# Peer222/art-sbir

Measured on AMD Instinct MI355X. Metric: triplet-images/sec embedded @224² bf16, 1→8 GPU; gallery kNN QPS @1M×512, higher is better.
Workload: dtype bf16; 1 GPU; triplet training step (train.py:59-70): 3x encoder fwd + TripletMarginLoss + backward + Adam; model=ModifiedResNet((3,4,6,3), output_dim=512), global_batch=384, triplets_per_gpu=384, resolution=224, parallelism=dp1

## Files before the change

### art-sbir_amd/csrc/bstream.hip

```cpp
#include "common.h"
#include "pgemm.h"
#include "pgemm_dev.h"
#include "../../include/artsbir.h"

namespace artsbir {

constexpr int BS_NW = 8;
constexpr int BS_KC = 4;
constexpr int BS_CHUNK = 64;
constexpr int BS_NSEGT = 2;
#ifndef ARTSBIR_BS_NT
#define ARTSBIR_BS_NT 0
#endif

#define BS_GLOBAL __attribute__((address_space(1)))
template <typename T>
__device__ __forceinline__ BS_GLOBAL T* bs_base(T* p, long long off) {
  return (BS_GLOBAL T*)pg_uniform((long long)(p + off));
}

typedef __attribute__((ext_vector_type(4))) unsigned bs_u4;
template <bool NT>
__device__ __forceinline__ void bs_store(BS_GLOBAL bf16* p, const Vec16<bf16>& v) {
  if constexpr (NT) __builtin_nontemporal_store(*reinterpret_cast<const bs_u4*>(&v), reinterpret_cast<BS_GLOBAL bs_u4*>(p));
  else *reinterpret_cast<BS_GLOBAL bs_u4*>(p) = *reinterpret_cast<const bs_u4*>(&v);
}

struct BsArgs {
  const bf16* y3;
  const bf16* res;
  const bf16* w;
  const float* bn3;
  const float* bnd;
  bf16* out;
  unsigned char* bits;
  bf16* y1;
  float* stats;
  int nblk;
  int seg_blk;
  int nseg;
  int chunk;
};

template <int K, int N, bool TWO>
__global__ void __launch_bounds__(BS_NW * 64) bstream_kernel(BsArgs a) {
  constexpr int CPR = K / 8;
  constexpr int NKC = K / (32 * BS_KC);
  constexpr int NT = N / 16;
  constexpr int NP = N / 32;
  constexpr int NQ = TWO ? 6 : 3;
  static_assert(NKC % 2 == 0, "two operand sets, a whole number of pairs per block");
  __shared__ __attribute__((aligned(16))) char wlds[N * K * 2];
  __shared__ __attribute__((aligned(16))) float prm[BS_NSEGT][NQ][K];

  const int tid = threadIdx.x, lane = tid & 63;
  const int wid = __builtin_amdgcn_readfirstlane(tid >> 6);
  const int fr = lane & 15, fq = lane >> 4;
  const int b0 = blockIdx.x * a.chunk;
  const int b1 = b0 + a.chunk < a.nblk ? b0 + a.chunk : a.nblk;
// ... 258 lines not shown
```

### art-sbir_amd/csrc/gemm.hip

```cpp
#include <cstdio>
#include <cstdlib>
#include <tuple>
#include <vector>

#include "common.h"
#include "conv_launch.h"
#include "pgemm.h"
#include "tune.h"

namespace artsbir {

typedef __attribute__((ext_vector_type(4))) unsigned int u32x4;
#define OOB_OFFSET 0x80000000u

__device__ __forceinline__ __amdgpu_buffer_rsrc_t make_rsrc(const void* base, long long bytes) {
  if (bytes > 0x7fffffffLL) bytes = 0x7fffffffLL;
  if (bytes < 0) bytes = 0;
  return __builtin_amdgcn_make_buffer_rsrc(const_cast<void*>(base), (short)0, (int)bytes, 0x00020000);
}
__device__ __forceinline__ uint4 bload(__amdgpu_buffer_rsrc_t r, unsigned off) {
  u32x4 v = __builtin_amdgcn_raw_buffer_load_b128(r, (int)off, 0, 0);
  return make_uint4(v[0], v[1], v[2], v[3]);
}

// ... 668 lines not shown
  if (!g_tune_stats.reserve(bd ? per * bd->ntarget : (a.stats ? per : 0))) return pgemm_default_cfg(p);
  ConvArgs at = a;
  PgArgs pt = p;
  artsbir_bn_bwd_desc bt;
  if (a.stats) { at.stats = g_tune_stats.p; pt.stats = g_tune_stats.p; }
  if (bd) {
    bt = *bd;
    for (int t = 0; t < bd->ntarget; ++t) { bt.slots[t] = g_tune_stats.p + t * per; pt.bnb_slots[t] = bt.slots[t]; }
    at.bnb_desc = &bt;
  }
  return tune::fastest(pgemm_tune_candidates(), -2, st, [&](int c) { return run_candidate(c, at, pt, st); });
}

template <typename T>
static int launch_conv(const ConvArgs& a, hipStream_t st) {
  if ((long long)a.Cout * a.K * sizeof(T) > 0x7fffffffLL) { set_error("conv: weight tensor too large"); return -1; }
  if (a.nseg < 1 || a.M % a.nseg || (a.M / a.nseg) % ((long long)a.Ho * a.Wo)) {
    set_error("conv: %d BN segments do not split %lld output pixels into whole images", a.nseg, a.M);
    return -1;
  }
  const bool bnb = a.bnb_desc != nullptr;
  if (sizeof(T) == 2 && !a.out_f32 && !a.accumulate && !a.in_scale && !((a.bias || a.relu) && a.stats)) {
    const PgArgs p = to_pg(a);
    if (a.wg_p) {
      if (!pg_fold_wg_launch(p, st)) return 1;
      ARTSBIR_CHECK_LAUNCH("pgemm");
      return 0;
    }
    int choice;
    const char* force = getenv("ARTSBIR_PGEMM_CFG");
    static const char* force_bnb = getenv("ARTSBIR_BNB_CFG");
    if (force || (bnb && force_bnb)) {
      choice = atoi(force ? force : force_bnb);
    } else {
      const ConvKey key{a.M, a.H, a.W, a.C, a.Cout, a.R, a.S, a.stride, a.pad, a.Ho, a.Wo, a.res_mode,
                        (a.stats ? 1 : 0) | (a.bias ? 2 : 0) | (a.relu ? 4 : 0) | (a.x2 ? 8 : 0), a.nseg,
                        bnb ? p.bnb * 4 + p.bnb_nt : 0};
      choice = g_conv_choice.choice(
          key, st,
          [&] {
            const int c = pgemm_default_cfg(p);
            return c < 0 ? -2 : c;
          },
          [&] { return tune_conv(a, p, st); });
    }
    if ((choice != -2 && pgemm_launch_cfg(p, choice, st)) || (bnb && force_bnb && pgemm_launch_cfg(p, 0, st))) {
      ARTSBIR_CHECK_LAUNCH("pgemm");
      return 0;
    }
  }
  if (a.res_mode == 3) { set_error("gemm_nt_gate: no kernel for this shape"); return -1; }
  if (a.x2 || a.wg_p) return 1;
  return run_old<T>(a, st);
}

int artsbir::conv_launch(int dtype, const ConvArgs& a, hipStream_t st) {
  return dtype == ARTSBIR_DT_BF16 ? launch_conv<bf16>(a, st) : launch_conv<float>(a, st);
}

extern "C" int artsbir_conv2d_fwd(const artsbir_conv_desc* d, const void* x, const void* w, void* y,
                                  long long ldy, int out_f32, int accumulate, const float* bias,
                                  const float* in_scale, const float* in_shift, int in_relu,
                                  float* stats, void* stream) {
  if (check_conv(d)) return -1;
  if (accumulate && !out_f32) { set_error("conv: accumulate requires f32 output"); return -1; }
  ConvArgs a = conv_args_nhwc(d, x, w, y);
// ... 259 lines not shown
```

### art-sbir_amd/csrc/pgemm.h

```cpp
#pragma once
#include <hip/hip_runtime.h>

#include <vector>

namespace artsbir {

struct PgArgs {
  const void* x;
  long long x_elems;
  long long sN, sH, sW;
  int H, W, C;
  int R, S, stride, pad;
  int Ho, Wo;
  const void* w;
  int Cout, K;
  long long M;
  void* y;
  long long ldy;
  float* stats;
  long long seg_m;
  long long seg_stride;
  const void* res;
  int res_mode;
  const float* bias;
// ... 67 lines not shown
inline long long pg_ntiles(const PgArgs& a, int bpx, int bch) {
  return ((a.M + bpx - 1) / bpx) * ((a.Cout + bch - 1) / bch);
}

inline bool pg_supported(const PgArgs& a, bool& multi) {
  if (a.Cout % 32 != 0 || a.M <= 0) return false;
  if (a.C % 64 == 0) multi = false;
  else if (a.C == 8 || a.C == 16 || a.C == 32) multi = true;
  else return false;
  if (a.R * a.S > 32 || a.K % 8 != 0) return false;
  if ((long long)a.Cout * a.K * 2 > 0x7fffffffLL) return false;
  const long long HoWo = (long long)a.Ho * a.Wo;
  if (((256 + HoWo - 1) / HoWo + 2) * a.sN * 2 > 0x7fffffffLL) return false;
  if (a.M > (1LL << 40)) return false;
  if (a.seg_m > 0 && (a.seg_m % 64 != 0 || a.seg_m < 256 || a.M % a.seg_m != 0)) return false;
  if (a.bnb && (a.stats || a.Cout % 8 != 0)) return false;
  return true;
}

bool pg_pf_launch(int c, const PgArgs& a, bool multi, hipStream_t st);
bool pg_glb_launch(const PgArgs& a, bool multi, hipStream_t st);
bool pg_glb2_launch(const PgArgs& a, bool multi, hipStream_t st);
bool pg_k32w8_launch(const PgArgs& a, bool multi, hipStream_t st);
bool pg_fold_launch(const PgArgs& a, int c, hipStream_t st);
bool pstream_plain_launch(const PgArgs& a, bool multi, hipStream_t st);
bool pstream_bnb_launch(const PgArgs& a, bool multi, hipStream_t st);
bool pstream_k32_launch(const PgArgs& a, bool multi, hipStream_t st);
bool pstream_fold_launch(const PgArgs& a, int c, hipStream_t st);
bool sconv_launch(const PgArgs& a, hipStream_t st);
bool sconv_ok(const PgArgs& a);
bool hconv_launch(const PgArgs& a, hipStream_t st);
bool pp256_launch(const PgArgs& a, bool persistent, hipStream_t st);
bool rstream_launch(const PgArgs& a, hipStream_t st);
inline bool pg_fold_ok(const PgArgs& a, int bpx, int ks) {
  if (!a.x2 && !a.w_sstride) return true;
  if (a.R != 1 || a.S != 1 || a.stride != 1 || a.pad != 0) return false;
  if (a.x2 && (a.C1 <= 0 || a.C1 % ks != 0 || a.C1 >= a.C || (a.C - a.C1) % 8 != 0)) return false;
  if ((a.w_sstride || a.bias_sstride) && a.seg_m > 0 && a.seg_m % bpx != 0) return false;
  return true;
}
bool pg_fold_wg_launch(const PgArgs& a, hipStream_t st);
int pgemm_default_cfg(const PgArgs& a);

}
```

### art-sbir_amd/csrc/conv3x3.hip

```cpp
#include <cstdio>

#include "pgemm.h"
#include "pgemm_dev.h"

namespace artsbir {

__device__ __forceinline__ int sc_sw(int rho) { return (rho ^ (rho >> 1)) & 3; }

template <int C, int COUT, int STRIDE, bool BNB>
__global__ void __launch_bounds__(256) sconv_kernel(PgArgs a, int ntiles) {
  constexpr int K = 9 * C;
  constexpr int NKK = (K + 31) / 32;
  constexpr int CPT = C / 8;
  constexpr int MTC = COUT / 16, NTP = 4, WTPX = 64, BPX = 256, BCH = COUT;
  constexpr int PF = 2;
  constexpr int WB = NKK * COUT * 64;
  __shared__ __attribute__((aligned(16))) char smem[WB + pg_red_bytes<BCH>()];
  float* red = reinterpret_cast<float*>(smem + WB);
  int* red_cnt = reinterpret_cast<int*>(smem + WB + 6 * BCH * 4);
  const int tid = threadIdx.x, lane = tid & 63;
  const int wid = __builtin_amdgcn_readfirstlane(tid >> 6);
  const int fr = lane & 15, fq = lane >> 4;
  const bool sums = a.stats != nullptr || a.bnb != 0;
  if (sums) {
// ... 122 lines not shown
  } else if (a.stride == 1 && a.C == 32 && a.Cout == 64) {
    set_last_kernel(BNB ? "sconv_kernel<32,64,bnb>" : "sconv_kernel<32,64>");
    hipLaunchKernelGGL((sconv_kernel<32, 64, 1, BNB>), dim3(sconv_grid<32, 64, 1, BNB>(ntiles)), dim3(256), 0, st, a, ntiles);
  } else if (a.stride == 1 && a.C == 64 && a.Cout == 32) {
    set_last_kernel(BNB ? "sconv_kernel<64,32,bnb>" : "sconv_kernel<64,32>");
    hipLaunchKernelGGL((sconv_kernel<64, 32, 1, BNB>), dim3(sconv_grid<64, 32, 1, BNB>(ntiles)), dim3(256), 0, st, a, ntiles);
  } else if (a.stride == 1 && a.C == 64 && a.Cout == 64) {
    set_last_kernel(BNB ? "sconv_kernel<64,64,bnb>" : "sconv_kernel<64,64>");
    hipLaunchKernelGGL((sconv_kernel<64, 64, 1, BNB>), dim3(sconv_grid<64, 64, 1, BNB>(ntiles)), dim3(256), 0, st, a, ntiles);
  } else if (a.stride == 2 && a.C == 8 && a.Cout == 32) {
    set_last_kernel(BNB ? "sconv_kernel<8,32,s2,bnb>" : "sconv_kernel<8,32,s2>");
    hipLaunchKernelGGL((sconv_kernel<8, 32, 2, BNB>), dim3(sconv_grid<8, 32, 2, BNB>(ntiles)), dim3(256), 0, st, a, ntiles);
  } else {
    return false;
  }
  return true;
}

bool sconv_launch(const PgArgs& a, hipStream_t st) {
  if (!sconv_ok(a)) return false;
  const int ntiles = (int)((a.M + 255) / 256);
  if (a.bnb) return sconv_dispatch<true>(a, ntiles, st);
  return sconv_dispatch<false>(a, ntiles, st);
}

#define HC_MAXSEG 4
template <int C>
__device__ __forceinline__ int hc_addr(int q, int c) {
  constexpr int PB = 64 / (C / 8);
  constexpr int PBL = PB == 16 ? 4 : 3;
  return ((q >> PBL) << 10) + c * (PB * 16) + ((q & (PB - 1)) << 4);
}

template <int C, int COUT, int TR, int TC>
struct HcGeom {
  static constexpr int NWC = 4;
  static constexpr int CPT = C / 8, PB = 64 / CPT;
  static constexpr int NKK = 9 * C / 32;
  static constexpr int MTC = COUT / 16, NP = MTC / 2;
  static constexpr int TCB = TC / 16;
  static constexpr int NTP = TR * TCB / NWC;
  static constexpr int HW = TC + 2, NQ = HW * (TR + 2);
  static constexpr int NB = (NQ + PB - 1) / PB;
  static constexpr int HB = NB * 1024;
  static constexpr int WB = NKK * COUT * 64;
  static constexpr int PRM = HC_MAXSEG * 4 * COUT * 4;
  static constexpr int FIX = WB + PRM + pg_red_bytes<COUT>();
  static constexpr bool THREE = FIX + 3 * HB <= 160 * 1024 && (160 * 1024) / (FIX + 3 * HB) ==
                                (160 * 1024) / (FIX + 2 * HB) && NB <= 31;
  static constexpr int NBUF = THREE ? 3 : 2;
  static constexpr int LDS = WB + NBUF * HB + PRM + pg_red_bytes<COUT>();
  static constexpr int WPB = (160 * 1024) / LDS > 4 ? 4 : (160 * 1024) / LDS;
  static constexpr int WPE = (5 * WPB + 3) / 4 > 3 ? 3 : (5 * WPB + 3) / 4;
};

template <int C, int COUT, int TR, int TC, bool BNB>
__global__ void __launch_bounds__(320) __attribute__((amdgpu_waves_per_eu(HcGeom<C, COUT, TR, TC>::WPE)))
hconv_kernel(PgArgs a, int ntiles) {
  using Gm = HcGeom<C, COUT, TR, TC>;
  constexpr int NWC = Gm::NWC, PB = Gm::PB, NKK = Gm::NKK, MTC = Gm::MTC, NP = Gm::NP;
  constexpr int TCB = Gm::TCB, NTP = Gm::NTP, HW = Gm::HW, NQ = Gm::NQ, NB = Gm::NB, HB = Gm::HB;
  constexpr int WB = Gm::WB, NBUF = Gm::NBUF;
  static_assert(C % 32 == 0 && COUT % 32 == 0 && TC % 16 == 0, "tile shape");
  static_assert(NTP * NWC == TR * TCB, "pixel tiles per wave");
  static_assert(Gm::LDS <= 160 * 1024, "LDS");
  __shared__ __attribute__((aligned(16))) char smem[Gm::LDS];
  float* prm = reinterpret_cast<float*>(smem + WB + NBUF * HB);
  float* red = reinterpret_cast<float*>(smem + WB + NBUF * HB + Gm::PRM);
  int* red_cnt = reinterpret_cast<int*>(smem + WB + NBUF * HB + Gm::PRM + 6 * COUT * 4);
  const int tid = threadIdx.x, lane = tid & 63;
  const int wid = __builtin_amdgcn_readfirstlane(tid >> 6);
  const int fr = lane & 15, fq = lane >> 4;
  const int G = gridDim.x;
  const int ntw = (a.Wo + TC - 1) / TC, nth = (a.Ho + TR - 1) / TR;
  const int HoWo = a.Ho * a.Wo;
  const bool sums = a.stats != nullptr || BNB;

  auto issue_halo = [&](int t, int buf) {
    const int img = t / (nth * ntw), rem = t - img * (nth * ntw);
    const int h0 = (rem / ntw) * TR, w0 = (rem - (rem / ntw) * ntw) * TC;
    const __amdgpu_buffer_rsrc_t xr =
        pg_rsrc(reinterpret_cast<const bf16*>(a.x) + (long long)img * a.sN, (a.x_elems - (long long)img * a.sN) * 2);
    char* hb = smem + WB + buf * HB;
    const int c = lane / PB, ql = lane - c * PB;
#pragma unroll 4
    for (int b = 0; b < NB; ++b) {
      const int q = b * PB + ql;
      const int hr = q / HW, hc = q - (q / HW) * HW;
      const int ih = h0 - 1 + hr, iw = w0 - 1 + hc;
      const bool ok = q < NQ && ih >= 0 && ih < a.H && iw >= 0 && iw < a.W;
      glds16(xr, hb + b * 1024, ok ? (unsigned)((ih * (int)a.sH + iw * (int)a.sW) * 2 + c * 16) : PG_OOB);
    }
  };

  if (wid == NWC) {
    if ((int)blockIdx.x < ntiles) issue_halo(blockIdx.x, 0);
    if (NBUF == 3 && (int)blockIdx.x + G < ntiles) issue_halo(blockIdx.x + G, 1);
  } else {
    if (sums) {
      for (int i = tid; i < 6 * COUT; i += 64 * NWC) red[i] = 0.f;
      if (tid == 0) *red_cnt = 0;
    }
    if constexpr (BNB) {
      const int nsg = a.seg_m > 0 ? (int)(a.M / a.seg_m) : 1;
      for (int i = tid; i < nsg * 4 * COUT; i += 64 * NWC) {
        const int sg = i / (4 * COUT), r = (i / COUT) & 3, ch = i % COUT;
        const float* src = r == 0 ? a.bnb_istd[0] : r == 1 ? a.bnb_mean[0]
                         : r == 2 ? a.bnb_mbn + 2 * a.Cout : a.bnb_mbn + 3 * a.Cout;
        prm[i] = src[sg * a.bnb_pstride + ch];
      }
    }
    for (int i = tid; i < NKK * COUT * 4; i += 64 * NWC) {
      const int kk = i / (COUT * 4), rem = i - kk * COUT * 4;
      const int rho = rem >> 2, c = rem & 3;
      const uint4 v =
          *reinterpret_cast<const uint4*>(reinterpret_cast<const bf16*>(a.w) + (long long)pg_perm(rho) * a.K + kk * 32 + c * 8);
      *reinterpret_cast<uint4*>(smem + (kk * COUT + rho) * 64 + ((c ^ sc_sw(rho)) << 4)) = v;
    }
  }

  if (wid == NWC) {
    int k = 0;
    for (int tile = blockIdx.x; tile < ntiles; tile += G, ++k) {
      if (NBUF == 3 && tile + G < ntiles) vm_wait<NB>();
      else vm_wait<0>();
      __builtin_amdgcn_s_barrier();
      asm volatile("" ::: "memory");
      if (tile + (NBUF - 1) * G < ntiles) issue_halo(tile + (NBUF - 1) * G, (k + NBUF - 1) % NBUF);
    }
    vm_wait<0>();
    return;
  }
  auto tile_px = [&](int tile, long long (&px)[NTP], bool (&pv)[NTP], int (&qb)[NTP]) {
    const int img = tile / (nth * ntw), rem = tile - img * (nth * ntw);
    const int h0 = (rem / ntw) * TR, w0 = (rem - (rem / ntw) * ntw) * TC;
    const long long pimg = (long long)img * HoWo;
#pragma unroll
    for (int j = 0; j < NTP; ++j) {
      const int m = wid * NTP + j, row = m / TCB, cb = m - (m / TCB) * TCB;
      const int oh = h0 + row, ow = w0 + cb * 16 + fr;
      pv[j] = oh < a.Ho && ow < a.Wo;
      px[j] = pv[j] ? pimg + oh * a.Wo + ow : pimg;
      qb[j] = row * HW + cb * 16 + fr;
    }
    return pimg;
  };
  Vec16<bf16> yp[NP][NTP];
  auto load_yp = [&](const long long (&px)[NTP]) {
#pragma unroll
    for (int p = 0; p < NP; ++p)
#pragma unroll
      for (int j = 0; j < NTP; ++j)
        yp[p][j] = ld16<bf16>(reinterpret_cast<const bf16*>(a.bnb_y[0]) + px[j] * a.ldy + 32 * p + 8 * fq);
  };
  if constexpr (BNB) {
    if ((int)blockIdx.x < ntiles) {
      long long px0[NTP];
      bool pv0[NTP];
      int qb0[NTP];
      tile_px(blockIdx.x, px0, pv0, qb0);
      load_yp(px0);
    }
  }
  int k = 0;
  for (int tile = blockIdx.x; tile < ntiles; tile += G, ++k) {
    asm volatile("s_waitcnt lgkmcnt(0)" ::: "memory");
    __builtin_amdgcn_s_barrier();
    asm volatile("" ::: "memory");
    long long px[NTP];
    bool pv[NTP];
    int qb[NTP];
    const long long pimg = tile_px(tile, px, pv, qb);
    const long long wseg = a.seg_m > 0 ? pimg / a.seg_m : 0;
    const char* hb = smem + WB + (k % NBUF) * HB;
    f32x4 acc[MTC][NTP];
#pragma unroll
    for (int i = 0; i < MTC; ++i)
#pragma unroll
      for (int j = 0; j < NTP; ++j) acc[i][j] = f32x4{0.f, 0.f, 0.f, 0.f};
    constexpr int KPT = C / 32;
    constexpr int TUN = ((NTP <= 2 || (C == 32 && MTC * NTP <= 8)) && !(Gm::WPE >= 3 && NTP > 2)) ? 9 : 3;
#pragma unroll TUN
    for (int t = 0; t < 9; ++t) {
      const int toff = (t / 3) * HW + (t % 3);
      int qa[NTP];
#pragma unroll
      for (int j = 0; j < NTP; ++j) qa[j] = qb[j] + toff;
#pragma unroll
    for (int h = 0; h < KPT; ++h) {
      const int kk = t * KPT + h, c = h * 4 + fq;
      uint4 af[MTC], bv[NTP];
#pragma unroll
      for (int i = 0; i < MTC; ++i) {
        const int rho = i * 16 + fr;
        af[i] = *reinterpret_cast<const uint4*>(smem + (kk * COUT + rho) * 64 + ((fq ^ sc_sw(rho)) << 4));
      }
#pragma unroll
      for (int j = 0; j < NTP; ++j) bv[j] = *reinterpret_cast<const uint4*>(hb + hc_addr<C>(qa[j], c));
#pragma unroll
      for (int i = 0; i < MTC; ++i)
#pragma unroll
        for (int j = 0; j < NTP; ++j)
          acc[i][j] = __builtin_amdgcn_mfma_f32_16x16x32_bf16(*reinterpret_cast<const bf16x8*>(&af[i]),
                                                              *reinterpret_cast<const bf16x8*>(&bv[j]), acc[i][j], 0, 0, 0);
    }
    }
#pragma unroll
    for (int p = 0; p < NP; ++p) {
      const int ch0 = 32 * p + 8 * fq;
      float s1[8], s2[8];
#pragma unroll
      for (int e = 0; e < 8; ++e) { s1[e] = 0.f; s2[e] = 0.f; }
      float xa[8], xm[8], ms[8], mh[8];
      if constexpr (BNB) {
        const float* pp = prm + wseg * 4 * COUT + ch0;
        loadf8v(pp, xa);
        loadf8v(pp + COUT, xm);
        loadf8v(pp + 2 * COUT, ms);
        loadf8v(pp + 3 * COUT, mh);
      }
#pragma unroll
      for (int j = 0; j < NTP; ++j) {
        float v[8];
#pragma unroll
        for (int r = 0; r < 4; ++r) { v[r] = acc[2 * p][j][r]; v[4 + r] = acc[2 * p + 1][j][r]; }
        if (pv[j]) {
          if constexpr (!BNB) {
            if (a.bias) {
#pragma unroll
              for (int e = 0; e < 8; ++e) v[e] += a.bias[ch0 + e];
            }
            if (a.relu) {
#pragma unroll
              for (int e = 0; e < 8; ++e) v[e] = fmaxf(v[e], 0.f);
            }
          }
          if constexpr (BNB) {
#pragma unroll
            for (int e = 0; e < 8; ++e) {
              const float yv = to_f(yp[p][j].v[e]);
              v[e] = (yv - xm[e]) * ms[e] + mh[e] > 0.f ? v[e] : 0.f;
              s1[e] += v[e];
              s2[e] += v[e] * ((yv - xm[e]) * xa[e]);
            }
          } else if (sums) {
#pragma unroll
            for (int e = 0; e < 8; ++e) { s1[e] += v[e]; s2[e] += v[e] * v[e]; }
          }
          Vec16<bf16> o;
#pragma unroll
          for (int e = 0; e < 8; ++e) o.v[e] = from_f<bf16>(v[e]);
          st16<bf16>(reinterpret_cast<bf16*>(a.y) + px[j] * a.ldy + ch0, o);
        }
      }
      if (sums) {
#pragma unroll
        for (int e = 0; e < 8; ++e) { s1[e] = dpp_row_sum(s1[e]); s2[e] = dpp_row_sum(s2[e]); }
        if (fr == 15) {
#pragma unroll
          for (int e = 0; e < 8; ++e) {
            atomicAdd(red + ch0 + e, s1[e]);
            atomicAdd(red + COUT + ch0 + e, s2[e]);
          }
        }
      }
    }
    if constexpr (BNB) {
      if (tile + G < ntiles) {
        long long pxn[NTP];
        bool pvn[NTP];
        int qbn[NTP];
        tile_px(tile + G, pxn, pvn, qbn);
        load_yp(pxn);
      }
    }
    if (sums) stats_flush<COUT>(red, red_cnt, NWC * (k + 1) - 1, a, 0, tile % ARTSBIR_NSLOT, lane, pimg, 1);
  }
}

static bool hconv_ok(const PgArgs& a) {
  if (a.R != 3 || a.S != 3 || a.pad != 1 || a.stride != 1 || a.M <= 0) return false;
  if ((a.C != 32 && a.C != 64) || (a.Cout != 32 && a.Cout != 64) || a.K != 9 * a.C) return false;
  if (a.res_mode || (a.bnb && (a.bnb != 1 || a.bnb_nt != 1 || a.stats))) return false;
  const long long HoWo = (long long)a.Ho * a.Wo;
  if (a.Ho != a.H || a.Wo != a.W || a.M % HoWo) return false;
  if (a.seg_m > 0 && (a.seg_m % HoWo || a.M % a.seg_m)) return false;
  if (a.bnb && a.seg_m > 0 && a.M / a.seg_m > HC_MAXSEG) return false;
  if (a.sW < a.C || a.sN * 2 > 0x7fffffffLL || (long long)a.H * a.sH * 2 > 0x7fffffffLL) return false;
  const long long nt = (a.M / HoWo) * ((a.Ho + 15) / 16) * ((a.Wo + 15) / 16) * 2;
  return nt < 0x7fffffffLL;
}

template <int C, int COUT, int TR, int TC, bool BNB>
static void hconv_go(const PgArgs& a, hipStream_t st) {
  using Gm = HcGeom<C, COUT, TR, TC>;
  const int ntiles = (int)((a.M / ((long long)a.Ho * a.Wo)) * ((a.Ho + TR - 1) / TR) * ((a.Wo + TC - 1) / TC));
  int per_cu = (160 * 1024) / Gm::LDS;
  if (per_cu > 4) per_cu = 4;
  const int g = 256 * per_cu < ntiles ? 256 * per_cu : ntiles;
  static const char* nm = nullptr;
  static char buf[64];
  if (!nm) {
    snprintf(buf, sizeof buf, "hconv_kernel<%d,%d,%dx%d%s>", C, COUT, TR, TC, BNB ? ",bnb" : "");
    nm = buf;
  }
  set_last_kernel(nm);
  hipLaunchKernelGGL((hconv_kernel<C, COUT, TR, TC, BNB>), dim3(g), dim3(320), 0, st, a, ntiles);
}

template <int C, int COUT, bool BNB>
static void hconv_tiles(const PgArgs& a, hipStream_t st) {
  if (a.Ho % 16 == 0 && a.Wo % 16 == 0) hconv_go<C, COUT, 16, 16, BNB>(a, st);
  else hconv_go<C, COUT, 8, 16, BNB>(a, st);
}

template <bool BNB>
static void hconv_dispatch(const PgArgs& a, hipStream_t st) {
  if (a.C == 32 && a.Cout == 32) hconv_tiles<32, 32, BNB>(a, st);
  else if (a.C == 32) hconv_tiles<32, 64, BNB>(a, st);
  else if (a.Cout == 32) hconv_tiles<64, 32, BNB>(a, st);
  else hconv_tiles<64, 64, BNB>(a, st);
}

bool hconv_launch(const PgArgs& a, hipStream_t st) {
  if (!hconv_ok(a)) return false;
  if (a.bnb) hconv_dispatch<true>(a, st);
  else hconv_dispatch<false>(a, st);
  return true;
}

}
```

Baseline: 13150 triplet-images/s.

## Add streaming 1x1 expansion-conv kernel with fused BN stats and resident weights

Adds a specialized streaming kernel for 1x1 stride-1 convolutions that expand channels 4x (C=128/256 to 4C) with BN statistics output. Each workgroup keeps a weight slice resident in swizzled LDS and streams 16-row pixel blocks with double-buffered register loads. MFMA outputs are stored directly, and per-channel sum and sum-of-squares are reduced via DPP and LDS before atomics into per-segment slots. It is dispatched ahead of the tuned pgemm path and bypasses autotuning, so it risks being slower than the tuned choice for some shapes. It also moves shared store helpers into a common header.

```diff
diff --git a/art-sbir_amd/csrc/bstream.hip b/art-sbir_amd/csrc/bstream.hip
--- a/art-sbir_amd/csrc/bstream.hip
+++ b/art-sbir_amd/csrc/bstream.hip
@@ -1,6 +1,7 @@
 #include "common.h"
 #include "pgemm.h"
 #include "pgemm_dev.h"
+#include "stream_io.h"
 #include "../../include/artsbir.h"
 
 namespace artsbir {
@@ -12,19 +13,6 @@
 #ifndef ARTSBIR_BS_NT
 #define ARTSBIR_BS_NT 0
 #endif
-
-#define BS_GLOBAL __attribute__((address_space(1)))
-template <typename T>
-__device__ __forceinline__ BS_GLOBAL T* bs_base(T* p, long long off) {
-  return (BS_GLOBAL T*)pg_uniform((long long)(p + off));
-}
-
-typedef __attribute__((ext_vector_type(4))) unsigned bs_u4;
-template <bool NT>
-__device__ __forceinline__ void bs_store(BS_GLOBAL bf16* p, const Vec16<bf16>& v) {
-  if constexpr (NT) __builtin_nontemporal_store(*reinterpret_cast<const bs_u4*>(&v), reinterpret_cast<BS_GLOBAL bs_u4*>(p));
-  else *reinterpret_cast<BS_GLOBAL bs_u4*>(p) = *reinterpret_cast<const bs_u4*>(&v);
-}
 
 struct BsArgs {
   const bf16* y3;
diff --git a/art-sbir_amd/csrc/cstream.hip b/art-sbir_amd/csrc/cstream.hip
--- /dev/null
+++ b/art-sbir_amd/csrc/cstream.hip
@@ -0,0 +1,231 @@
+#include "common.h"
+#include "pgemm.h"
+#include "pgemm_dev.h"
+#include "stream_io.h"
+#include "../../include/artsbir.h"
+
+namespace artsbir {
+
+constexpr int CS_CHUNK = 256;
+
+struct CsArgs {
+  const bf16* x;
+  const bf16* w;
+  bf16* y;
+  float* stats;
+  int nblk;
+  int seg_blk;
+  int chunk;
+};
+
+template <int K, int NS, int NB, int NW>
+__global__ void __launch_bounds__(NW * 64) cstream_kernel(CsArgs a) {
+  constexpr int N = 4 * K;
+  constexpr int CPR = K / 8;
+  constexpr int KS = K / 32;
+  constexpr int NP = NS / 32;
+  constexpr int PG = NB == 1 ? 2 : 1;
+  static_assert(CPR >= 16 && N % NS == 0 && NP % PG == 0, "the swizzle needs 16 chunks per row; whole slices, whole passes");
+  __shared__ __attribute__((aligned(16))) char wlds[NS * K * 2];
+  __shared__ float red[2 * NS];
+
+  const int tid = threadIdx.x, lane = tid & 63;
+  const int wid = __builtin_amdgcn_readfirstlane(tid >> 6);
+  const int fr = lane & 15, fq = lane >> 4;
+  constexpr int NSL = N / NS;
+  const long long lid = pg_xcd_remap(blockIdx.x, (long long)gridDim.x);
+  const int n0 = (int)(lid % NSL) * NS, grp = (int)(lid / NSL);
+  const int b0 = grp * a.chunk;
+  const int b1 = b0 + a.chunk < a.nblk ? b0 + a.chunk : a.nblk;
+
+  for (int i = tid; i < NS * CPR; i += NW * 64) {
+    const int rho = i / CPR, c = i - rho * CPR;
+    const uint4 v = *reinterpret_cast<const uint4*>(a.w + (long long)(n0 + pg_perm(rho)) * K + c * 8);
+    *reinterpret_cast<uint4*>(wlds + (rho * CPR + (c ^ (rho & 15))) * 16) = v;
+  }
+  for (int i = tid; i < 2 * NS; i += NW * 64) red[i] = 0.f;
+  __syncthreads();
+
+  const bf16* const xp = a.x;
+  bf16* const yp = a.y;
+  float* const statp = a.stats;
+  const int seg_blk = a.seg_blk;
+  const int slot = grp % ARTSBIR_NSLOT;
+  const unsigned lof = fr * K + 8 * fq, lo1 = fr * N + n0 + 8 * fq;
+  const int lx = fq ^ fr;
+
+  float s1[NP][8], s2[NP][8];
+  auto zero_sums = [&]() __attribute__((always_inline)) {
+#pragma unroll
+    for (int p = 0; p < NP; ++p)
+#pragma unroll
+      for (int e = 0; e < 8; ++e) { s1[p][e] = 0.f; s2[p][e] = 0.f; }
+  };
+  zero_sums();
+  auto flush = [&](int seg) __attribute__((always_inline)) {
+#pragma unroll
+    for (int p = 0; p < NP; ++p) {
+#pragma unroll
+      for (int e = 0; e < 8; ++e) { s1[p][e] = dpp_row_sum(s1[p][e]); s2[p][e] = dpp_row_sum(s2[p][e]); }
+      if (fr == 15) {
+#pragma unroll
+        for (int e = 0; e < 8; ++e) {
+          atomicAdd(&red[32 * p + 8 * fq + e], s1[p][e]);
+          atomicAdd(&red[NS + 32 * p + 8 * fq + e], s2[p][e]);
+        }
+      }
+    }
+    zero_sums();
+    __syncthreads();
+    float* so = statp + ((long long)seg * ARTSBIR_NSLOT + slot) * 2 * N + n0;
+    const int t0 = 64 * wid + (int)__builtin_amdgcn_mbcnt_hi(~0u, __builtin_amdgcn_mbcnt_lo(~0u, 0u));
+    for (int i = t0; i < 2 * NS; i += NW * 64) {
+      const int h = i / NS, c = i - h * NS;
+      atomicAdd(so + h * N + c, red[i]);
+      red[i] = 0.f;
+    }
+    __syncthreads();
+  };
+
+  auto load = [&](int blk, bs_u4 (&xv)[NB][KS]) __attribute__((always_inline)) {
+#pragma unroll
+    for (int b = 0; b < NB; ++b) {
+      const BS_GLOBAL bf16* xblk = bs_base(xp, (long long)(blk + b) * 16 * K);
+#pragma unroll
+      for (int s = 0; s < KS; ++s) xv[b][s] = *reinterpret_cast<const BS_GLOBAL bs_u4*>(xblk + (lof + 32 * s));
+    }
+  };
+  auto compute = [&](int blk, const bs_u4 (&xv)[NB][KS]) __attribute__((always_inline)) {
+    int wrow = fr * CPR * 16;
+    asm volatile("" : "+v"(wrow));
+    BS_GLOBAL bf16* yblk[NB];
+#pragma unroll
+    for (int b = 0; b < NB; ++b) yblk[b] = bs_base(yp, (long long)(blk + b) * 16 * N);
+#pragma unroll
+    for (int p0 = 0; p0 < NP; p0 += PG) {
+      f32x4 acc[2 * PG][NB];
+#pragma unroll
+      for (int i = 0; i < 2 * PG; ++i)
+#pragma unroll
+        for (int b = 0; b < NB; ++b) acc[i][b] = f32x4{0.f, 0.f, 0.f, 0.f};
+#pragma unroll
+      for (int s = 0; s < KS; ++s) {
+        uint4 af[2 * PG];
+#pragma unroll
+        for (int i = 0; i < 2 * PG; ++i)
+          af[i] = *reinterpret_cast<const uint4*>(wlds + wrow + (16 * (2 * p0 + i) * CPR + 4 * (s & ~3) + ((4 * (s & 3)) ^ lx)) * 16);
+#pragma unroll
+        for (int i = 0; i < 2 * PG; ++i)
+#pragma unroll
+          for (int b = 0; b < NB; ++b)
+            acc[i][b] = __builtin_amdgcn_mfma_f32_16x16x32_bf16(*reinterpret_cast<const bf16x8*>(&af[i]),
+                                                                *reinterpret_cast<const bf16x8*>(&xv[b][s]),
+                                                                acc[i][b], 0, 0, 0);
+      }
+#pragma unroll
+      for (int q = 0; q < PG; ++q)
+#pragma unroll
+        for (int b = 0; b < NB; ++b) {
+          const int p = p0 + q;
+          Vec16<bf16> ov;
+#pragma unroll
+          for (int e = 0; e < 8; ++e) {
+            const float v = acc[2 * q + (e >> 2)][b][e & 3];
+            s1[p][e] += v;
+            s2[p][e] += v * v;
+            ov.v[e] = from_f<bf16>(v);
+          }
+          bs_store<false>(yblk[b] + (lo1 + 32 * p), ov);
+        }
+      __builtin_amdgcn_sched_barrier(0);
+    }
+  };
+
+  constexpr int STEP = NW * NB;
+  bs_u4 xc[NB][KS], xn[NB][KS];
+  int blk = b0 + wid * NB;
+  if (blk < b1) load(blk, xc);
+  int seg = b0 / seg_blk;
+#pragma nounroll
+  for (int ph = 0; ph < 2; ++ph, ++seg) {
+    const int seg_end = (seg + 1) * seg_blk;
+    const int lim = seg_end < b1 ? seg_end : b1;
+#pragma nounroll
+    while (blk < lim) {
+      int nxt = blk + STEP;
+      if (nxt < b1) load(nxt, xn);
+      compute(blk, xc);
+      blk = nxt;
+      if (blk >= lim) {
+#pragma unroll
+        for (int b = 0; b < NB; ++b)
+#pragma unroll
+          for (int s = 0; s < KS; ++s) xc[b][s] = xn[b][s];
+        break;
+      }
+      nxt = blk + STEP;
+      if (nxt < b1) load(nxt, xc);
+      compute(blk, xn);
+      blk = nxt;
+    }
+    flush(seg);
+    if (seg_end >= b1) break;
+  }
+}
+
+static int cstream_cus() {
+  static const int n = [] {
+    int dev = 0, v = 0;
+    if (hipGetDevice(&dev) != hipSuccess ||
+        hipDeviceGetAttribute(&v, hipDeviceAttributeMultiprocessorCount, dev) != hipSuccess || v <= 0)
+      v = 256;
+    return v;
+  }();
+  return n;
+}
+
+static bool cstream_on() {
+  const char* e = getenv("ARTSBIR_CSTREAM");
+  return !e || atoi(e) != 0;
+}
+
+template <int K, int NS, int NB, int NW>
+static bool cs_go(CsArgs a, const char* name, hipStream_t st) {
+  constexpr int N = 4 * K;
+  if (a.seg_blk % NB) return false;
+  const int nsl = N / NS, cus = cstream_cus();
+  long long wgs = (long long)((a.nblk + CS_CHUNK - 1) / CS_CHUNK) * nsl;
+  wgs = (wgs + cus - 1) / cus * cus;
+  long long grps = wgs / nsl > 0 ? wgs / nsl : 1;
+  long long chunk = (a.nblk + grps - 1) / grps;
+  chunk = (chunk + NB - 1) / NB * NB;
+  if (chunk > a.seg_blk) chunk = a.seg_blk;
+  a.chunk = (int)chunk;
+  grps = (a.nblk + chunk - 1) / chunk;
+  const dim3 g((unsigned)(grps * nsl)), b(NW * 64);
+  hipLaunchKernelGGL((cstream_kernel<K, NS, NB, NW>), g, b, 0, st, a);
+  set_last_kernel(name);
+  return true;
+}
+
+bool cstream_launch(const PgArgs& p, hipStream_t st) {
+  if (!p.stats || p.bnb || p.res || p.res_mode || p.bias || p.relu || p.x2 || p.w_sstride || p.wg_p) return false;
+  if (p.R != 1 || p.S != 1 || p.stride != 1 || p.pad != 0 || p.Cout != 4 * p.C || p.K != p.C) return false;
+  if (p.C != 128 && p.C != 256) return false;
+  if (p.sW != p.C || p.sH != (long long)p.W * p.C || p.sN != (long long)p.H * p.W * p.C || p.ldy != p.Cout) return false;
+  if (p.x_elems < p.M * p.C) return false;
+  const long long seg_m = p.seg_m > 0 ? p.seg_m : p.M;
+  if (p.M <= 0 || p.M % seg_m || seg_m % 16 != 0 || p.M / 16 > 0x3fffffffLL) return false;
+  if (!cstream_on()) return false;
+  CsArgs a;
+  a.x = reinterpret_cast<const bf16*>(p.x);
+  a.w = reinterpret_cast<const bf16*>(p.w);
+  a.y = reinterpret_cast<bf16*>(p.y);
+  a.stats = p.stats;
+  a.nblk = (int)(p.M / 16); a.seg_blk = (int)(seg_m / 16); a.chunk = 0;
+  if (p.C == 128) return cs_go<128, 512, 1, 4>(a, "cstream_kernel<128,512>", st);
+  return cs_go<256, 256, 2, 4>(a, "cstream_kernel<256,256>", st) ||
+         cs_go<256, 128, 1, 8>(a, "cstream_kernel<256,128,one>", st);
+}
+
+}
diff --git a/art-sbir_amd/csrc/gemm.hip b/art-sbir_amd/csrc/gemm.hip
--- a/art-sbir_amd/csrc/gemm.hip
+++ b/art-sbir_amd/csrc/gemm.hip
@@ -724,6 +724,9 @@
     static const char* force_bnb = getenv("ARTSBIR_BNB_CFG");
     if (force || (bnb && force_bnb)) {
       choice = atoi(force ? force : force_bnb);
+    } else if (cstream_launch(p, st)) {
+      ARTSBIR_CHECK_LAUNCH("cstream");
+      return 0;
     } else {
       const ConvKey key{a.M, a.H, a.W, a.C, a.Cout, a.R, a.S, a.stride, a.pad, a.Ho, a.Wo, a.res_mode,
                         (a.stats ? 1 : 0) | (a.bias ? 2 : 0) | (a.relu ? 4 : 0) | (a.x2 ? 8 : 0), a.nseg,
diff --git a/art-sbir_amd/csrc/pgemm.h b/art-sbir_amd/csrc/pgemm.h
--- a/art-sbir_amd/csrc/pgemm.h
+++ b/art-sbir_amd/csrc/pgemm.h
@@ -123,6 +123,7 @@
 bool hconv_launch(const PgArgs& a, hipStream_t st);
 bool pp256_launch(const PgArgs& a, bool persistent, hipStream_t st);
 bool rstream_launch(const PgArgs& a, hipStream_t st);
+bool cstream_launch(const PgArgs& a, hipStream_t st);
 inline bool pg_fold_ok(const PgArgs& a, int bpx, int ks) {
   if (!a.x2 && !a.w_sstride) return true;
   if (a.R != 1 || a.S != 1 || a.stride != 1 || a.pad != 0) return false;
diff --git a/art-sbir_amd/csrc/stream_io.h b/art-sbir_amd/csrc/stream_io.h
--- /dev/null
+++ b/art-sbir_amd/csrc/stream_io.h
@@ -0,0 +1,20 @@
+#pragma once
+#include "common.h"
+#include "pgemm_dev.h"
+
+namespace artsbir {
+
+#define BS_GLOBAL __attribute__((address_space(1)))
+template <typename T>
+__device__ __forceinline__ BS_GLOBAL T* bs_base(T* p, long long off) {
+  return (BS_GLOBAL T*)pg_uniform((long long)(p + off));
+}
+
+typedef __attribute__((ext_vector_type(4))) unsigned bs_u4;
+template <bool NT>
+__device__ __forceinline__ void bs_store(BS_GLOBAL bf16* p, const Vec16<bf16>& v) {
+  if constexpr (NT) __builtin_nontemporal_store(*reinterpret_cast<const bs_u4*>(&v), reinterpret_cast<BS_GLOBAL bs_u4*>(p));
+  else *reinterpret_cast<BS_GLOBAL bs_u4*>(p) = *reinterpret_cast<const bs_u4*>(&v);
+}
+
+}
```

Result: no change. 13280 triplet-images/s (median of 6 runs) (+1.0%).

## Restructure halo conv into two ping-pong compute groups with shared halo loading

Applied to the files above, without the earlier changes.

Replaces the dedicated producer wave plus four compute waves with 8 waves split into two groups that alternate tiles, with all waves cooperatively issuing halo loads into a fixed triple buffer. BN statistics are accumulated in registers across tiles and flushed straight to global slots with atomics, rather than per tile through an LDS reduction and stats_flush. When LDS is tight, the BN parameters are kept in registers. The goal is to overlap compute with loads and cut per-tile reduction and sync overhead, at the cost of higher register pressure and a more involved barrier protocol.

```diff
diff --git a/art-sbir_amd/csrc/conv3x3.hip b/art-sbir_amd/csrc/conv3x3.hip
--- a/art-sbir_amd/csrc/conv3x3.hip
+++ b/art-sbir_amd/csrc/conv3x3.hip
@@ -178,59 +178,55 @@
   return ((q >> PBL) << 10) + c * (PB * 16) + ((q & (PB - 1)) << 4);
 }
 
-template <int C, int COUT, int TR, int TC>
+template <int C, int COUT, int TR, int TC, bool BNB>
 struct HcGeom {
-  static constexpr int NWC = 4;
+  static constexpr int NWG = 4;
   static constexpr int CPT = C / 8, PB = 64 / CPT;
   static constexpr int NKK = 9 * C / 32;
   static constexpr int MTC = COUT / 16, NP = MTC / 2;
   static constexpr int TCB = TC / 16;
-  static constexpr int NTP = TR * TCB / NWC;
+  static constexpr int NTP = TR * TCB / NWG;
   static constexpr int HW = TC + 2, NQ = HW * (TR + 2);
   static constexpr int NB = (NQ + PB - 1) / PB;
   static constexpr int HB = NB * 1024;
   static constexpr int WB = NKK * COUT * 64;
-  static constexpr int PRM = HC_MAXSEG * 4 * COUT * 4;
-  static constexpr int FIX = WB + PRM + pg_red_bytes<COUT>();
-  static constexpr bool THREE = FIX + 3 * HB <= 160 * 1024 && (160 * 1024) / (FIX + 3 * HB) ==
-                                (160 * 1024) / (FIX + 2 * HB) && NB <= 31;
-  static constexpr int NBUF = THREE ? 3 : 2;
-  static constexpr int LDS = WB + NBUF * HB + PRM + pg_red_bytes<COUT>();
-  static constexpr int WPB = (160 * 1024) / LDS > 4 ? 4 : (160 * 1024) / LDS;
-  static constexpr int WPE = (5 * WPB + 3) / 4 > 3 ? 3 : (5 * WPB + 3) / 4;
+  static constexpr int PTAB = BNB ? HC_MAXSEG * 4 * COUT * 4 : 0;
+  static constexpr bool PREG = BNB && NP == 1 && WB + 3 * HB + PTAB > 160 * 1024;
+  static constexpr int PRM = PREG ? 0 : PTAB;
+  static constexpr int LDS = WB + 3 * HB + PRM;
+  static constexpr bool FITS = LDS <= 160 * 1024;
 };
 
 template <int C, int COUT, int TR, int TC, bool BNB>
-__global__ void __launch_bounds__(320) __attribute__((amdgpu_waves_per_eu(HcGeom<C, COUT, TR, TC>::WPE)))
-hconv_kernel(PgArgs a, int ntiles) {
-  using Gm = HcGeom<C, COUT, TR, TC>;
-  constexpr int NWC = Gm::NWC, PB = Gm::PB, NKK = Gm::NKK, MTC = Gm::MTC, NP = Gm::NP;
+__global__ void __launch_bounds__(512) hconv_kernel(PgArgs a, int ntiles) {
+  using Gm = HcGeom<C, COUT, TR, TC, BNB>;
+  constexpr int NWG = Gm::NWG, PB = Gm::PB, NKK = Gm::NKK, MTC = Gm::MTC, NP = Gm::NP;
   constexpr int TCB = Gm::TCB, NTP = Gm::NTP, HW = Gm::HW, NQ = Gm::NQ, NB = Gm::NB, HB = Gm::HB;
-  constexpr int WB = Gm::WB, NBUF = Gm::NBUF;
+  constexpr int WB = Gm::WB;
   static_assert(C % 32 == 0 && COUT % 32 == 0 && TC % 16 == 0, "tile shape");
-  static_assert(NTP * NWC == TR * TCB, "pixel tiles per wave");
-  static_assert(Gm::LDS <= 160 * 1024, "LDS");
+  static_assert(NTP * NWG == TR * TCB, "pixel tiles per wave");
+  static_assert(Gm::FITS, "LDS");
   __shared__ __attribute__((aligned(16))) char smem[Gm::LDS];
-  float* prm = reinterpret_cast<float*>(smem + WB + NBUF * HB);
-  float* red = reinterpret_cast<float*>(smem + WB + NBUF * HB + Gm::PRM);
-  int* red_cnt = reinterpret_cast<int*>(smem + WB + NBUF * HB + Gm::PRM + 6 * COUT * 4);
+  float* prm = reinterpret_cast<float*>(smem + WB + 3 * HB);
   const int tid = threadIdx.x, lane = tid & 63;
   const int wid = __builtin_amdgcn_readfirstlane(tid >> 6);
+  const int grp = wid >> 2, wg = wid & 3;
   const int fr = lane & 15, fq = lane >> 4;
   const int G = gridDim.x;
   const int ntw = (a.Wo + TC - 1) / TC, nth = (a.Ho + TR - 1) / TR;
   const int HoWo = a.Ho * a.Wo;
   const bool sums = a.stats != nullptr || BNB;
-
-  auto issue_halo = [&](int t, int buf) {
+  const int n = (ntiles - (int)blockIdx.x + G - 1) / G;
+
+  auto issue_halo = [&](int j) {
+    const int t = blockIdx.x + j * G;
     const int img = t / (nth * ntw), rem = t - img * (nth * ntw);
     const int h0 = (rem / ntw) * TR, w0 = (rem - (rem / ntw) * ntw) * TC;
     const __amdgpu_buffer_rsrc_t xr =
         pg_rsrc(reinterpret_cast<const bf16*>(a.x) + (long long)img * a.sN, (a.x_elems - (long long)img * a.sN) * 2);
-    char* hb = smem + WB + buf * HB;
+    char* hb = smem + WB + (j % 3) * HB;
     const int c = lane / PB, ql = lane - c * PB;
-#pragma unroll 4
-    for (int b = 0; b < NB; ++b) {
+    for (int b = wg; b < NB; b += NWG) {
       const int q = b * PB + ql;
       const int hr = q / HW, hc = q - (q / HW) * HW;
       const int ih = h0 - 1 + hr, iw = w0 - 1 + hc;
@@ -239,126 +235,157 @@
     }
   };
 
-  if (wid == NWC) {
-    if ((int)blockIdx.x < ntiles) issue_halo(blockIdx.x, 0);
-    if (NBUF == 3 && (int)blockIdx.x + G < ntiles) issue_halo(blockIdx.x + G, 1);
-  } else {
-    if (sums) {
-      for (int i = tid; i < 6 * COUT; i += 64 * NWC) red[i] = 0.f;
-      if (tid == 0) *red_cnt = 0;
-    }
-    if constexpr (BNB) {
-      const int nsg = a.seg_m > 0 ? (int)(a.M / a.seg_m) : 1;
-      for (int i = tid; i < nsg * 4 * COUT; i += 64 * NWC) {
-        const int sg = i / (4 * COUT), r = (i / COUT) & 3, ch = i % COUT;
-        const float* src = r == 0 ? a.bnb_istd[0] : r == 1 ? a.bnb_mean[0]
-                         : r == 2 ? a.bnb_mbn + 2 * a.Cout : a.bnb_mbn + 3 * a.Cout;
-        prm[i] = src[sg * a.bnb_pstride + ch];
-      }
-    }
-    for (int i = tid; i < NKK * COUT * 4; i += 64 * NWC) {
-      const int kk = i / (COUT * 4), rem = i - kk * COUT * 4;
-      const int rho = rem >> 2, c = rem & 3;
-      const uint4 v =
-          *reinterpret_cast<const uint4*>(reinterpret_cast<const bf16*>(a.w) + (long long)pg_perm(rho) * a.K + kk * 32 + c * 8);
-      *reinterpret_cast<uint4*>(smem + (kk * COUT + rho) * 64 + ((c ^ sc_sw(rho)) << 4)) = v;
-    }
-  }
-
-  if (wid == NWC) {
-    int k = 0;
-    for (int tile = blockIdx.x; tile < ntiles; tile += G, ++k) {
-      if (NBUF == 3 && tile + G < ntiles) vm_wait<NB>();
-      else vm_wait<0>();
-      __builtin_amdgcn_s_barrier();
-      asm volatile("" ::: "memory");
-      if (tile + (NBUF - 1) * G < ntiles) issue_halo(tile + (NBUF - 1) * G, (k + NBUF - 1) % NBUF);
-    }
-    vm_wait<0>();
-    return;
-  }
-  auto tile_px = [&](int tile, long long (&px)[NTP], bool (&pv)[NTP], int (&qb)[NTP]) {
+  if (grp < n) issue_halo(grp);
+  if constexpr (BNB && !Gm::PREG) {
+    const int nsg = a.seg_m > 0 ? (int)(a.M / a.seg_m) : 1;
+    for (int i = tid; i < nsg * 4 * COUT; i += 128 * NWG) {
+      const int sg = i / (4 * COUT), r = (i / COUT) & 3, ch = i % COUT;
+      const float* src = r == 0 ? a.bnb_istd[0] : r == 1 ? a.bnb_mean[0]
+                       : r == 2 ? a.bnb_mbn + 2 * a.Cout : a.bnb_mbn + 3 * a.Cout;
+      prm[i] = src[sg * a.bnb_pstride + ch];
+    }
+  }
+  for (int i = tid; i < NKK * COUT * 4; i += 128 * NWG) {
+    const int kk = i / (COUT * 4), rem = i - kk * COUT * 4;
+    const int rho = rem >> 2, c = rem & 3;
+    const uint4 v =
+        *reinterpret_cast<const uint4*>(reinterpret_cast<const bf16*>(a.w) + (long long)pg_perm(rho) * a.K + kk * 32 + c * 8);
+    *reinterpret_cast<uint4*>(smem + (kk * COUT + rho) * 64 + ((c ^ sc_sw(rho)) << 4)) = v;
+  }
+  vm_wait<0>();
+
+  auto tile_px = [&](int j, long long (&px)[NTP], bool (&pv)[NTP], int (&qb)[NTP]) {
+    const int tile = blockIdx.x + j * G;
     const int img = tile / (nth * ntw), rem = tile - img * (nth * ntw);
     const int h0 = (rem / ntw) * TR, w0 = (rem - (rem / ntw) * ntw) * TC;
     const long long pimg = (long long)img * HoWo;
 #pragma unroll
-    for (int j = 0; j < NTP; ++j) {
-      const int m = wid * NTP + j, row = m / TCB, cb = m - (m / TCB) * TCB;
+    for (int m = 0; m < NTP; ++m) {
+      const int mt = wg * NTP + m, row = mt / TCB, cb = mt - (mt / TCB) * TCB;
       const int oh = h0 + row, ow = w0 + cb * 16 + fr;
-      pv[j] = oh < a.Ho && ow < a.Wo;
-      px[j] = pv[j] ? pimg + oh * a.Wo + ow : pimg;
-      qb[j] = row * HW + cb * 16 + fr;
+      pv[m] = oh < a.Ho && ow < a.Wo;
+      px[m] = pv[m] ? pimg + oh * a.Wo + ow : pimg;
+      qb[m] = row * HW + cb * 16 + fr;
     }
     return pimg;
   };
   Vec16<bf16> yp[NP][NTP];
-  auto load_yp = [&](const long long (&px)[NTP]) {
+  auto load_yp = [&](int j) {
+    long long px[NTP];
+    bool pv[NTP];
+    int qb[NTP];
+    tile_px(j, px, pv, qb);
 #pragma unroll
     for (int p = 0; p < NP; ++p)
 #pragma unroll
-      for (int j = 0; j < NTP; ++j)
-        yp[p][j] = ld16<bf16>(reinterpret_cast<const bf16*>(a.bnb_y[0]) + px[j] * a.ldy + 32 * p + 8 * fq);
+      for (int m = 0; m < NTP; ++m)
+        yp[p][m] = ld16<bf16>(reinterpret_cast<const bf16*>(a.bnb_y[0]) + px[m] * a.ldy + 32 * p + 8 * fq);
   };
   if constexpr (BNB) {
-    if ((int)blockIdx.x < ntiles) {
-      long long px0[NTP];
-      bool pv0[NTP];
-      int qb0[NTP];
-      tile_px(blockIdx.x, px0, pv0, qb0);
-      load_yp(px0);
-    }
-  }
-  int k = 0;
-  for (int tile = blockIdx.x; tile < ntiles; tile += G, ++k) {
+    if (grp < n) load_yp(grp);
+  }
+  float cs1[NP][8], cs2[NP][8];
+#pragma unroll
+  for (int p = 0; p < NP; ++p)
+#pragma unroll
+    for (int e = 0; e < 8; ++e) { cs1[p][e] = 0.f; cs2[p][e] = 0.f; }
+  long long cseg = -1;
+  float preg[4][8];
+  const int slot = (int)((blockIdx.x * (2 * NWG) + wid) % ARTSBIR_NSLOT);
+  auto sums_flush = [&]() {
+    const long long so = cseg * a.seg_stride + (long long)slot * 2 * a.Cout;
+    float* dst = (BNB ? a.bnb_slots[0] : a.stats) + so;
+#pragma unroll
+    for (int p = 0; p < NP; ++p) {
+      const int ch0 = 32 * p + 8 * fq;
+#pragma unroll
+      for (int e = 0; e < 8; ++e) { cs1[p][e] = dpp_row_sum(cs1[p][e]); cs2[p][e] = dpp_row_sum(cs2[p][e]); }
+      if (fr == 15 && !(a.dbg & 1)) {
+#pragma unroll
+        for (int e = 0; e < 8; ++e) {
+          atomicAdd(dst + ch0 + e, cs1[p][e]);
+          atomicAdd(dst + a.Cout + ch0 + e, cs2[p][e]);
+        }
+      }
+#pragma unroll
+      for (int e = 0; e < 8; ++e) { cs1[p][e] = 0.f; cs2[p][e] = 0.f; }
+    }
+  };
+  auto barrier = [&]() {
     asm volatile("s_waitcnt lgkmcnt(0)" ::: "memory");
     __builtin_amdgcn_s_barrier();
     asm volatile("" ::: "memory");
+  };
+
+  if (grp == 1) {
+    barrier();
+    if (2 < n) issue_halo(2);
+  }
+  for (int j = grp; j < n; j += 2) {
+    barrier();
     long long px[NTP];
     bool pv[NTP];
     int qb[NTP];
-    const long long pimg = tile_px(tile, px, pv, qb);
+    const long long pimg = tile_px(j, px, pv, qb);
     const long long wseg = a.seg_m > 0 ? pimg / a.seg_m : 0;
-    const char* hb = smem + WB + (k % NBUF) * HB;
+    const char* hb = smem + WB + (j % 3) * HB;
     f32x4 acc[MTC][NTP];
 #pragma unroll
     for (int i = 0; i < MTC; ++i)
 #pragma unroll
-      for (int j = 0; j < NTP; ++j) acc[i][j] = f32x4{0.f, 0.f, 0.f, 0.f};
+      for (int m = 0; m < NTP; ++m) acc[i][m] = f32x4{0.f, 0.f, 0.f, 0.f};
     constexpr int KPT = C / 32;
-    constexpr int TUN = ((NTP <= 2 || (C == 32 && MTC * NTP <= 8)) && !(Gm::WPE >= 3 && NTP > 2)) ? 9 : 3;
+    constexpr int TUN = (NTP <= 2 || (C == 32 && MTC * NTP <= 8)) ? 9 : 3;
 #pragma unroll TUN
     for (int t = 0; t < 9; ++t) {
       const int toff = (t / 3) * HW + (t % 3);
       int qa[NTP];
 #pragma unroll
-      for (int j = 0; j < NTP; ++j) qa[j] = qb[j] + toff;
-#pragma unroll
-    for (int h = 0; h < KPT; ++h) {
-      const int kk = t * KPT + h, c = h * 4 + fq;
-      uint4 af[MTC], bv[NTP];
-#pragma unroll
-      for (int i = 0; i < MTC; ++i) {
-        const int rho = i * 16 + fr;
-        af[i] = *reinterpret_cast<const uint4*>(smem + (kk * COUT + rho) * 64 + ((fq ^ sc_sw(rho)) << 4));
-      }
-#pragma unroll
-      for (int j = 0; j < NTP; ++j) bv[j] = *reinterpret_cast<const uint4*>(hb + hc_addr<C>(qa[j], c));
-#pragma unroll
-      for (int i = 0; i < MTC; ++i)
-#pragma unroll
-        for (int j = 0; j < NTP; ++j)
-          acc[i][j] = __builtin_amdgcn_mfma_f32_16x16x32_bf16(*reinterpret_cast<const bf16x8*>(&af[i]),
-                                                              *reinterpret_cast<const bf16x8*>(&bv[j]), acc[i][j], 0, 0, 0);
-    }
+      for (int m = 0; m < NTP; ++m) qa[m] = qb[m] + toff;
+#pragma unroll
+      for (int h = 0; h < KPT; ++h) {
+        const int kk = t * KPT + h, c = h * 4 + fq;
+        uint4 af[MTC], bv[NTP];
+#pragma unroll
+        for (int i = 0; i < MTC; ++i) {
+          const int rho = i * 16 + fr;
+          af[i] = *reinterpret_cast<const uint4*>(smem + (kk * COUT + rho) * 64 + ((fq ^ sc_sw(rho)) << 4));
+        }
+#pragma unroll
+        for (int m = 0; m < NTP; ++m) bv[m] = *reinterpret_cast<const uint4*>(hb + hc_addr<C>(qa[m], c));
+#pragma unroll
+        for (int i = 0; i < MTC; ++i)
+#pragma unroll
+          for (int m = 0; m < NTP; ++m)
+            acc[i][m] = __builtin_amdgcn_mfma_f32_16x16x32_bf16(*reinterpret_cast<const bf16x8*>(&af[i]),
+                                                                *reinterpret_cast<const bf16x8*>(&bv[m]), acc[i][m], 0, 0, 0);
+      }
+    }
+    vm_wait<0>();
+    barrier();
+    if (j + 3 < n) issue_halo(j + 3);
+    if (sums && wseg != cseg) {
+      if (cseg >= 0) sums_flush();
+      cseg = wseg;
+      if constexpr (Gm::PREG) {
+        const long long po = wseg * a.bnb_pstride + 8 * fq;
+#pragma unroll
+        for (int e = 0; e < 8; ++e) {
+          preg[0][e] = a.bnb_istd[0][po + e];
+          preg[1][e] = a.bnb_mean[0][po + e];
+          preg[2][e] = a.bnb_mbn[2 * a.Cout + po + e];
+          preg[3][e] = a.bnb_mbn[3 * a.Cout + po + e];
+        }
+      }
     }
 #pragma unroll
     for (int p = 0; p < NP; ++p) {
       const int ch0 = 32 * p + 8 * fq;
-      float s1[8], s2[8];
-#pragma unroll
-      for (int e = 0; e < 8; ++e) { s1[e] = 0.f; s2[e] = 0.f; }
       float xa[8], xm[8], ms[8], mh[8];
-      if constexpr (BNB) {
+      if constexpr (Gm::PREG) {
+#pragma unroll
+        for (int e = 0; e < 8; ++e) { xa[e] = preg[0][e]; xm[e] = preg[1][e]; ms[e] = preg[2][e]; mh[e] = preg[3][e]; }
+      } else if constexpr (BNB) {
         const float* pp = prm + wseg * 4 * COUT + ch0;
         loadf8v(pp, xa);
         loadf8v(pp + COUT, xm);
@@ -366,11 +393,11 @@
         loadf8v(pp + 3 * COUT, mh);
       }
 #pragma unroll
-      for (int j = 0; j < NTP; ++j) {
+      for (int m = 0; m < NTP; ++m) {
         float v[8];
 #pragma unroll
-        for (int r = 0; r < 4; ++r) { v[r] = acc[2 * p][j][r]; v[4 + r] = acc[2 * p + 1][j][r]; }
-        if (pv[j]) {
+        for (int r = 0; r < 4; ++r) { v[r] = acc[2 * p][m][r]; v[4 + r] = acc[2 * p + 1][m][r]; }
+        if (pv[m]) {
           if constexpr (!BNB) {
             if (a.bias) {
 #pragma unroll
@@ -384,44 +411,28 @@
           if constexpr (BNB) {
 #pragma unroll
             for (int e = 0; e < 8; ++e) {
-              const float yv = to_f(yp[p][j].v[e]);
+              const float yv = to_f(yp[p][m].v[e]);
               v[e] = (yv - xm[e]) * ms[e] + mh[e] > 0.f ? v[e] : 0.f;
-              s1[e] += v[e];
-              s2[e] += v[e] * ((yv - xm[e]) * xa[e]);
+              cs1[p][e] += v[e];
+              cs2[p][e] += v[e] * ((yv - xm[e]) * xa[e]);
             }
           } else if (sums) {
 #pragma unroll
-            for (int e = 0; e < 8; ++e) { s1[e] += v[e]; s2[e] += v[e] * v[e]; }
+            for (int e = 0; e < 8; ++e) { cs1[p][e] += v[e]; cs2[p][e] += v[e] * v[e]; }
           }
           Vec16<bf16> o;
 #pragma unroll
           for (int e = 0; e < 8; ++e) o.v[e] = from_f<bf16>(v[e]);
-          st16<bf16>(reinterpret_cast<bf16*>(a.y) + px[j] * a.ldy + ch0, o);
+          st16<bf16>(reinterpret_cast<bf16*>(a.y) + px[m] * a.ldy + ch0, o);
         }
       }
-      if (sums) {
-#pragma unroll
-        for (int e = 0; e < 8; ++e) { s1[e] = dpp_row_sum(s1[e]); s2[e] = dpp_row_sum(s2[e]); }
-        if (fr == 15) {
-#pragma unroll
-          for (int e = 0; e < 8; ++e) {
-            atomicAdd(red + ch0 + e, s1[e]);
-            atomicAdd(red + COUT + ch0 + e, s2[e]);
-          }
-        }
-      }
     }
     if constexpr (BNB) {
-      if (tile + G < ntiles) {
-        long long pxn[NTP];
-        bool pvn[NTP];
-        int qbn[NTP];
-        tile_px(tile + G, pxn, pvn, qbn);
-        load_yp(pxn);
-      }
-    }
-    if (sums) stats_flush<COUT>(red, red_cnt, NWC * (k + 1) - 1, a, 0, tile % ARTSBIR_NSLOT, lane, pimg, 1);
-  }
+      if (j + 2 < n) load_yp(j + 2);
+    }
+  }
+  if (((n + grp) & 1) == 0) barrier();
+  if (sums && cseg >= 0) sums_flush();
 }
 
 static bool hconv_ok(const PgArgs& a) {
@@ -439,10 +450,17 @@
 
 template <int C, int COUT, int TR, int TC, bool BNB>
 static void hconv_go(const PgArgs& a, hipStream_t st) {
-  using Gm = HcGeom<C, COUT, TR, TC>;
+  using Gm = HcGeom<C, COUT, TR, TC, BNB>;
   const int ntiles = (int)((a.M / ((long long)a.Ho * a.Wo)) * ((a.Ho + TR - 1) / TR) * ((a.Wo + TC - 1) / TC));
-  int per_cu = (160 * 1024) / Gm::LDS;
-  if (per_cu > 4) per_cu = 4;
+  static const int per_cu = [] {
+    int n = (160 * 1024) / Gm::LDS;
+    if (n > 4) n = 4;
+    int occ = 0;
+    if (hipOccupancyMaxActiveBlocksPerMultiprocessor(&occ, hconv_kernel<C, COUT, TR, TC, BNB>, 512, 0) == hipSuccess &&
+        occ >= 1 && occ < n)
+      n = occ;
+    return n;
+  }();
   const int g = 256 * per_cu < ntiles ? 256 * per_cu : ntiles;
   static const char* nm = nullptr;
   static char buf[64];
@@ -451,13 +469,15 @@
     nm = buf;
   }
   set_last_kernel(nm);
-  hipLaunchKernelGGL((hconv_kernel<C, COUT, TR, TC, BNB>), dim3(g), dim3(320), 0, st, a, ntiles);
+  hipLaunchKernelGGL((hconv_kernel<C, COUT, TR, TC, BNB>), dim3(g), dim3(512), 0, st, a, ntiles);
 }
 
 template <int C, int COUT, bool BNB>
 static void hconv_tiles(const PgArgs& a, hipStream_t st) {
-  if (a.Ho % 16 == 0 && a.Wo % 16 == 0) hconv_go<C, COUT, 16, 16, BNB>(a, st);
-  else hconv_go<C, COUT, 8, 16, BNB>(a, st);
+  if constexpr (HcGeom<C, COUT, 16, 16, BNB>::FITS) {
+    if (a.Ho % 16 == 0 && a.Wo % 16 == 0) return hconv_go<C, COUT, 16, 16, BNB>(a, st);
+  }
+  hconv_go<C, COUT, 8, 16, BNB>(a, st);
 }
 
 template <bool BNB>
```

After: 12950 triplet-images/s before, 13190 triplet-images/s after (median of 6 runs). 1.02x the previous value.
